# ccuchengwei/LongReadSelfCorrect

Measured on NVIDIA B200. Metric: corrected Mbp/s (seed + FM-extend + DP/MSA fallback, default options), higher is better.
Workload: dtype int64+f64

## Files before the change

longreadselfcorrect_b200/csrc/fm_table.cuh:

```cuda
#ifndef PBSC_FM_TABLE_CUH
#define PBSC_FM_TABLE_CUH

#include <cuda_runtime.h>
#include <stdint.h>

namespace pbsc {

struct __align__(32) FmBlock
{
    uint32_t cnt[4];
    uint32_t bases[4];
};

struct __align__(32) PrefixEntry
{
    uint64_t fwd_lo, rvc_lo;
    uint32_t fwd_size, rvc_size;
    uint32_t pad[2];
};

struct FmTable
{
    const FmBlock* blocks;
    const uint32_t* dollar_pos;
// ... 42 lines not shown
__host__ __device__ __forceinline__ uint32_t count_dollars(const FmTable& t, uint64_t from, uint64_t to)
{
    uint32_t lo = 0, hi = t.n_dollar;
    while (lo < hi) { uint32_t m = (lo + hi) >> 1; if ((uint64_t)PBSC_LDG(t.dollar_pos + m) < from) lo = m + 1; else hi = m; }
    uint32_t a = lo;
    hi = t.n_dollar;
    while (lo < hi) { uint32_t m = (lo + hi) >> 1; if ((uint64_t)PBSC_LDG(t.dollar_pos + m) < to) lo = m + 1; else hi = m; }
    return lo - a;
}

__host__ __device__ __forceinline__ uint64_t occ(const FmTable& t, int c, uint64_t p)
{
    PBSC_OCC_TICK(1);
    const uint64_t blk = p >> 6;
    const uint32_t off = (uint32_t)p & 63u;
    const uint4* bp = reinterpret_cast<const uint4*>(t.blocks + blk);
    const uint4 cn = PBSC_LDG(bp);
    const uint4 bs = PBSC_LDG(bp + 1);
    uint32_t base = c == 0 ? cn.x : c == 1 ? cn.y : c == 2 ? cn.z : cn.w;
    const bool has_dollar = (cn.x >> 31) != 0;
    if (c == 0) base &= 0x7fffffffu;
    const uint64_t w0 = (uint64_t)bs.x | ((uint64_t)bs.y << 32);
    const uint64_t w1 = (uint64_t)bs.z | ((uint64_t)bs.w << 32);
    const uint64_t pat = 0x5555555555555555ull * (uint64_t)c;
    uint64_t x0 = w0 ^ pat, x1 = w1 ^ pat;
    uint64_t m0 = ~(x0 | (x0 >> 1)) & 0x5555555555555555ull;
    uint64_t m1 = ~(x1 | (x1 >> 1)) & 0x5555555555555555ull;
    if (off < 32) { m0 &= (1ull << (2 * off)) - 1ull; m1 = 0; }
    else { m1 &= (1ull << (2 * (off - 32))) - 1ull; }
    uint64_t r = (uint64_t)base + PBSC_POPCLL(m0) + PBSC_POPCLL(m1);
    if (c == 0 && has_dollar && off) r -= PBSC_POPCLL(PBSC_LDG(t.dollar_mask + blk) & ((1ull << off) - 1ull));
    return r;
}

__host__ __device__ __forceinline__ void occ4(const FmTable& t, uint64_t p, uint64_t r[4])
{
    PBSC_OCC_TICK(1);
    const uint64_t blk = p >> 6;
    const uint32_t off = (uint32_t)p & 63u;
    const uint4* bp = reinterpret_cast<const uint4*>(t.blocks + blk);
    const uint4 cn = PBSC_LDG(bp);
    const uint4 bs = PBSC_LDG(bp + 1);
    const uint64_t w0 = (uint64_t)bs.x | ((uint64_t)bs.y << 32);
    const uint64_t w1 = (uint64_t)bs.z | ((uint64_t)bs.w << 32);
    const uint64_t M = 0x5555555555555555ull;
    uint64_t k0, k1;
    if (off < 32) { k0 = ((1ull << (2 * off)) - 1ull) & M; k1 = 0; }
    else { k0 = M; k1 = ((1ull << (2 * (off - 32))) - 1ull) & M; }
    const uint64_t l0 = w0 & M, h0 = (w0 >> 1) & M, l1 = w1 & M, h1 = (w1 >> 1) & M;
    const uint32_t nT = PBSC_POPCLL(h0 & l0 & k0) + PBSC_POPCLL(h1 & l1 & k1);
    const uint32_t nG = PBSC_POPCLL(h0 & ~l0 & k0) + PBSC_POPCLL(h1 & ~l1 & k1);
    const uint32_t nC = PBSC_POPCLL(~h0 & l0 & k0) + PBSC_POPCLL(~h1 & l1 & k1);
    uint32_t nA = off - nT - nG - nC;
    if ((cn.x >> 31) && off) nA -= PBSC_POPCLL(PBSC_LDG(t.dollar_mask + blk) & ((1ull << off) - 1ull));
    r[0] = (uint64_t)(cn.x & 0x7fffffffu) + nA;
    r[1] = (uint64_t)cn.y + nC;
    r[2] = (uint64_t)cn.z + nG;
    r[3] = (uint64_t)cn.w + nT;
}

__host__ __device__ __forceinline__ void occ_pair(const FmTable& t, int c, uint64_t lo, uint64_t hi, uint64_t& a, uint64_t& b)
{
    if ((lo >> 6) != (hi >> 6)) { a = occ(t, c, lo); b = occ(t, c, hi); return; }
    PBSC_OCC_TICK(1);
    const uint64_t blk = lo >> 6;
    const uint32_t off_a = (uint32_t)lo & 63u, off_b = (uint32_t)hi & 63u;
// ... 106 lines not shown
```

longreadselfcorrect_b200/csrc/pbsc_extend_thread.cu:

```cuda
#include <cub/cub.cuh>
#include <stdlib.h>
#include <string.h>
#include <algorithm>
#include <chrono>
#include "pbsc_batch.cuh"
#include "pbsc_task.cuh"
#include "pbsc_dp.cuh"

namespace pbsc {

constexpr int TW_BLOCK = 128;
struct ReadState
{
    int32_t t, next, started, done, rstatus, firstType;
    int32_t srcEnd, srcEndBest, srcRepeat;
    uint32_t nPieces;
    int64_t srcLen;
    uint64_t plen;
    int32_t pending_trg;
    int32_t srcFreq;
    int32_t srcStart;
    uint32_t nLog;
    int32_t dpStatus0;
    uint32_t dpLen0;
// ... 168 lines not shown
                                              : (y < (uint32_t)(k + interval) ? pth[y - k] : trgS[y - k - interval]);
            v.q[x] = 3 - c;
        }
    }
    tw::setup_task(idx, P, v, qlen, (uint32_t)k, interval, trgLen, tk.out_cap);
}

#ifdef PBSC_STAGE_CLOCKS
#define PBSC_N_STAGE 24
__device__ unsigned long long g_stage_clk[PBSC_N_STAGE];
#define STAGE_BEGIN() long long stg_t = clock64(); unsigned long long stg_acc[12] = {0, 0, 0, 0, 0, 0, 0, 0, 0, 0, 0, 0}
#define STAGE_MARK(i) do { const long long stg_n = clock64(); stg_acc[i] += (unsigned long long)(stg_n - stg_t); stg_t = stg_n; } while (0)
#define STAGE_COUNT(i, v) do { const unsigned stg_v = __reduce_add_sync(FULL, (unsigned)(v)); stg_acc[i] += stg_v; } while (0)
#define STAGE_END() do { if ((threadIdx.x & 31) == 0) for (int stg_i = 0; stg_i < 12; stg_i++) atomicAdd(&g_stage_clk[stg_i], stg_acc[stg_i]); } while (0)
#else
#define STAGE_BEGIN()
#define STAGE_MARK(i)
#define STAGE_COUNT(i, v)
#define STAGE_END()
#endif

__device__ __forceinline__ void
walk_levels_body(const FmIndexDev& idx, const ExtParamsDev& P, uint8_t* scratch, size_t stride,
                   unsigned long long* counter, uint64_t n_items, const uint32_t* __restrict__ list, WalkTask* tasks, uint8_t* recpool,
                   const uint64_t* __restrict__ rec_off, uint64_t pend_base, uint64_t pend_cap, uint8_t* outpool, uint64_t minSA,
                   unsigned long long* walk_counter, uint32_t* heavy_list, unsigned int* n_heavy, uint32_t* nodepool,
                   unsigned long long* pool_used, uint64_t pool_cap, tw::Caps caps, const unsigned int* n_items_dev, int last_pass, int owners)
{
    const bool owner = (int)(threadIdx.x & 31) < owners;
    const size_t tid = (((size_t)blockIdx.x * blockDim.x + threadIdx.x) >> 5) * (size_t)owners + (threadIdx.x & 31);
    __shared__ tw::Lane lanes_all[TW_BLOCK];
    tw::Lane* ctx = lanes_all + (threadIdx.x & ~31u);
    tw::Lane& S = ctx[threadIdx.x & 31];
    const tw::Layout Y = tw::make_layout(P.node_cap, caps);
    uint8_t* const my_scratch = scratch + (owner ? tid : 0) * stride;
    if (n_items_dev) n_items = *n_items_dev;
    S.status = 0; S.n = 0;
    WalkTask* tk = nullptr;
    tw::SetupHdr* hdr = nullptr;
    constexpr int REFILL_BATCH = 1;
    bool active = false, ended = false, exhausted = !owner;
    unsigned long long done = 0;
    STAGE_BEGIN();
    for (;;)
    {
        const unsigned waiting = __ballot_sync(FULL, !active && !exhausted);
        const unsigned walking = __ballot_sync(FULL, active);
        if (waiting && (__popc(waiting) >= REFILL_BATCH || !walking))
        {
            if (ended)
            {
                uint32_t mlen = 0;
                int st = tw::finish_walk(S, Y, P, hdr, nodepool, pool_used, pool_cap, last_pass != 0, outpool + tk->out_off, tk->out_cap, &mlen);
                if (st == PBSC_WALK_HEAVY && last_pass) st = PBSC_OVF_TREE;
                tk->out_len = st == 1 ? mlen : 0;
                tk->status = st;
                if (st == PBSC_WALK_HEAVY) heavy_list[atomicAdd(n_heavy, 1u)] = (uint32_t)(tk - tasks);
                ended = false;
            }
            if (!active && !exhausted)
            {
                for (;;)
                {
                    const unsigned long long it = atomicAdd(counter, 1ull);
                    if (it >= n_items) { exhausted = true; break; }
                    const uint64_t ti = list ? list[it] : it;
                    tk = &tasks[ti];
// ... 5 lines not shown
                    tw::begin_walk(S, Y, P, my_scratch, v, minSA);
                    hdr = v.hdr;
                    active = true;
                    done++;
                    break;
                }
            }
        }
        if (__all_sync(FULL, !active)) break;
        STAGE_MARK(0);
        const bool lv = active && tw::walk_continues(S, P);
        {
            const bool need = lv && tw::needs_refine(S);
            STAGE_COUNT(9, 1u);
            STAGE_COUNT(10, lv ? 1u : 0u);
            STAGE_COUNT(11, lv ? S.n : 0u);
            tw::refine_pool(idx, Y, ctx, need ? S.n : 0u);
            if (need) S.curK = S.maxOverlap;
        }
        STAGE_MARK(1);
        if (lv)
        {
            tw::filter_leaves(S, Y);
            S.thr = S.phase == 2 ? S.minSA - 1 : S.minSA;
        }
        STAGE_MARK(2);
        tw::pool_run(lv ? S.n : 0u, [&](int owner_lane, uint32_t i) { tw::probe_leaf(idx, Y, ctx[owner_lane], i); });
        STAGE_MARK(3);
        uint32_t m = 0, sel = 0;
        bool go = false;
        if (lv)
        {
            m = tw::adopt_children(S, Y);
            if (S.status == 0) go = tw::level_middle(S, Y, P, m, sel);
        }
        STAGE_MARK(4);
        if (__any_sync(FULL, sel != 0))
        {
            tw::pool_run(sel, [&](int owner_lane, uint32_t i) { tw::select_leaf(idx, Y, ctx[owner_lane], i); });
            if (sel) tw::level_select(S, P);
            tw::pool_run(sel, [&](int owner_lane, uint32_t i) { tw::reselect_leaf(idx, Y, ctx[owner_lane], i); });
        }
        STAGE_MARK(5);
        tw::pool_run(go ? m : 0u, [&](int owner_lane, uint32_t j) { tw::prune_leaf(P, Y, ctx[owner_lane], j); });
        STAGE_MARK(6);
        bool check_term = false;
        if (go) { S.level++; check_term = S.curLen >= S.minLength; }
        tw::pool_run(check_term ? m : 0u, [&](int owner_lane, uint32_t j) { tw::term_leaf(Y, ctx[owner_lane], j); });
        STAGE_MARK(7);
        if (go) tw::finish_level(S, Y, P, m, check_term);
        if (active && !tw::walk_continues(S, P)) { active = false; ended = true; }
        STAGE_MARK(8);
    }
    STAGE_END();
    if (done) atomicAdd(walk_counter, done);
}

template <int MINB>
__global__ void __launch_bounds__(TW_BLOCK, MINB)
walk_levels_kernel(const __grid_constant__ FmIndexDev idx, const __grid_constant__ ExtParamsDev P, uint8_t* scratch, size_t stride,
                   unsigned long long* counter, uint64_t n_items, const uint32_t* __restrict__ list, WalkTask* tasks, uint8_t* recpool,
                   const uint64_t* __restrict__ rec_off, uint64_t pend_base, uint64_t pend_cap, uint8_t* outpool, uint64_t minSA,
                   unsigned long long* walk_counter, uint32_t* heavy_list, unsigned int* n_heavy, uint32_t* nodepool,
                   unsigned long long* pool_used, uint64_t pool_cap, tw::Caps caps, const unsigned int* n_items_dev, int last_pass, int owners)
{
    walk_levels_body(idx, P, scratch, stride, counter, n_items, list, tasks, recpool, rec_off, pend_base, pend_cap, outpool, minSA, walk_counter,
                     heavy_list, n_heavy, nodepool, pool_used, pool_cap, caps, n_items_dev, last_pass, owners);
// ... 610 lines not shown
```

longreadselfcorrect_b200/csrc/pbsc_walk_thread.cuh:

```cuda
#ifndef PBSC_WALK_THREAD_CUH
#define PBSC_WALK_THREAD_CUH

#include "pbsc_walk.cuh"

namespace pbsc {
namespace tw {

struct Caps { uint32_t old_cap, new_cap, rings, res; };
#define PBSC_WALK_HEAVY (-102)

struct Layout
{
    uint32_t bank1, rings, nodes, res, ringStack, list0, list1;
    uint32_t node_cap;
    Caps cap;
};

__host__ __device__ inline uint32_t pow2_ceil(uint32_t x) { uint32_t p = 1; while (p < x) p <<= 1; return p; }

__host__ __device__ inline size_t thread_scratch_bytes(uint32_t node_cap, Caps c)
{
    size_t b = 0;
    b += sizeof(Leaf) * (size_t)(2 * c.new_cap);
    b += sizeof(double) * (size_t)c.rings * RING_LEN;
// ... 15 lines not shown
    y.ringStack = (uint32_t)p; p += align_up(c.rings, 16);
    y.list0 = (uint32_t)p; p += align_up(c.new_cap, 16);
    y.list1 = (uint32_t)p;
    y.node_cap = node_cap; y.cap = c;
    return y;
}

struct __align__(16) Lane
{
    uint8_t* base;
    const uint16_t* start4; const uint16_t* pos4; const uint8_t* q;
    const uint64_t* hash; const uint64_t* sF; const uint64_t* sR;
    const Interval* termF; const Interval* termR;
    double minErr;
    uint32_t curLen, curK, maxLength, minLength, maxIndel, minSA, thr;
    uint32_t qlen, k, maxOverlap, trgLen, nTerm, n9F, n9R, n5, nNodes, nRes, level, hashMask, nFree, nFresh, phase, n;
    uint32_t selLB, selExtra, selK;
    int selMx[3];
    int status;
    uint8_t dup, flip, selNew, pad;
};
static_assert(sizeof(Lane) == 208, "Lane: 208 bytes of shared memory per thread");

__device__ __forceinline__ Leaf* old_bank(const Lane& s, const Layout& y) { return (Leaf*)(s.base + (s.flip ? y.bank1 : 0u)); }
__device__ __forceinline__ Leaf* new_bank(const Lane& s, const Layout& y) { return (Leaf*)(s.base + (s.flip ? 0u : y.bank1)); }
__device__ __forceinline__ uint8_t* old_list(const Lane& s, const Layout& y) { return s.base + (s.flip ? y.list1 : y.list0); }
__device__ __forceinline__ uint8_t* new_list(const Lane& s, const Layout& y) { return s.base + (s.flip ? y.list0 : y.list1); }
__device__ __forceinline__ double* rings_of(const Lane& s, const Layout& y) { return (double*)(s.base + y.rings); }
__device__ __forceinline__ uint32_t* nodes_of(const Lane& s, const Layout& y) { return (uint32_t*)(s.base + y.nodes); }
__device__ __forceinline__ WalkResult* res_of(const Lane& s, const Layout& y) { return (WalkResult*)(s.base + y.res); }
__device__ __forceinline__ uint8_t* ring_stack(const Lane& s, const Layout& y) { return s.base + y.ringStack; }

static __device__ __noinline__ Interval update1(const FmTable& t, Interval iv, int c) { return update_interval(t, iv, c); }
static __device__ __noinline__ void occ4_ool(const FmTable& t, uint64_t p, uint64_t r[4]) { occ4(t, p, r); }
__device__ __forceinline__ void leaf_copy(Leaf* dst, const Leaf* src)
{
    const uint4* s4 = reinterpret_cast<const uint4*>(src);
    uint4* d4 = reinterpret_cast<uint4*>(dst);
    #pragma unroll
    for (int x = 0; x < (int)(sizeof(Leaf) / 16); x++) d4[x] = s4[x];
}

template <class Get>
__device__ __forceinline__ void both_strands(const FmIndexDev& idx, Get get, int K, Interval& f, Interval& r)
{
    int j;
    if (idx.prefix != nullptr && K >= idx.k0)
    {
        uint64_t key = 0;
        #pragma unroll 1
        for (int i = 0; i < idx.k0; i++) key |= (uint64_t)get(i) << (2 * i);
        prefix_lookup(idx, key, f, r);
        j = idx.k0;
    }
    else
    {
        const int c = get(0);
        f = init_interval(idx.t[PBSC_RBWT], c);
        r = init_interval(idx.t[PBSC_BWT], 3 - c);
        j = 1;
    }
    #pragma unroll 1
    for (; j < K && (f.valid() || r.valid()); j++)
    {
        const int c = get(j);
        if (f.valid()) f = update1(idx.t[PBSC_RBWT], f, c);
        if (r.valid()) r = update1(idx.t[PBSC_BWT], r, 3 - c);
    }
}

template <class F>
__device__ __forceinline__ void pool_run(uint32_t cnt, F f)
{
    __syncwarp();
// ... 27 lines not shown
}

__device__ __forceinline__ void ring_release(Lane& S, const Layout& Y, uint32_t slot) { ring_stack(S, Y)[S.nFree++] = (uint8_t)slot; }
__device__ __forceinline__ int ring_take(Lane& S, const Layout& Y)
{
    if (S.nFree) return (int)ring_stack(S, Y)[--S.nFree];
    return S.nFresh < Y.cap.rings ? (int)S.nFresh++ : -1;
}

__device__ __forceinline__ void refine_pool(const FmIndexDev& idx, const Layout& Y, const Lane* ctx, uint32_t cnt)
{
    pool_run(cnt, [&](int owner, uint32_t i) {
        const Lane& c = ctx[owner];
        Leaf* L = old_bank(c, Y) + old_list(c, Y)[i];
        const uint64_t rhi = L->rt_hi, rlo = L->rt_lo;
        const int K = (int)c.maxOverlap;
        Interval f, r;
        both_strands(idx, [&](int j) { return tail_base(rhi, rlo, K - 1 - j); }, K, f, r);
        L->f_lo = f.lo; L->f_hi = f.hi; L->r_lo = r.lo; L->r_hi = r.hi;
    });
}

__device__ __forceinline__ bool insufficient(const ExtParamsDev& P, const Leaf* bank, const uint8_t* list, uint32_t cnt)
{
    uint32_t high = 0;
    #pragma unroll 1
    for (uint32_t j = 0; j < cnt; j++) high += bank[list[j]].kmerFreq > P.high_freq_thr;
    if (high == 0) return true;
    if (high <= 2 && cnt >= 5) return true;
    if (high <= 1 && cnt >= 3) return true;
    return false;
}

static __device__ __noinline__ uint32_t eval4(const int freq[4], uint64_t totalcount, int maxfreq, uint32_t match5, uint32_t tailCount, uint64_t cutoffSA)
{
    uint32_t mask = 0;
    if (maxfreq <= 0) return 0;
    const bool isHomopolymer = tailCount >= 3;
    const bool isRepeat = maxfreq > 100, isHighlyRepeat = maxfreq > 150, isLowlyRepeat = maxfreq > 50;
    const bool isLowCoverage = totalcount >= cutoffSA + 2;
    #pragma unroll 1
    for (int b = 0; b < 4; b++)
    {
        const uint64_t kmerFreq = (uint64_t)(int64_t)freq[b];
        const bool isMatchedBy5mer = (match5 >> b) & 1;
        const bool isFreqPass = kmerFreq >= cutoffSA;
        int p, q;
        if (isMatchedBy5mer && isHighlyRepeat) { p = 1; q = 8; }
        else if (isMatchedBy5mer && isLowlyRepeat) { p = 1; q = 5; }
        else if (isFreqPass) { p = 1; q = 4; }
        else if (isLowCoverage) { p = 3; q = 5; }
        else { p = 2; q = 1; }
        if (isHomopolymer && isRepeat) { if (p * 10 < 3 * q) { p = 3; q = 10; } }
        else if (isHomopolymer) { if (p * 5 < 3 * q) { p = 3; q = 5; } }
        if ((int64_t)freq[b] * q >= (int64_t)p * maxfreq) mask |= 1u << b;
    }
    return mask;
}

__device__ __forceinline__ uint32_t match5_mask(const Lane& c, uint32_t tail4)
{
    const int64_t lo = max((int64_t)c.curLen - (int64_t)c.maxIndel, (int64_t)0);
    const int64_t hi = min((int64_t)c.curLen + (int64_t)c.maxIndel, (int64_t)c.n5 - 1);
    uint32_t mask = 0;
    const uint32_t e1 = c.start4[tail4 + 1];
    #pragma unroll 1
    for (uint32_t e = c.start4[tail4]; e < e1; e++)
    {
        const int64_t p = c.pos4[e];
        if (p >= lo && p <= hi) mask |= 1u << c.q[p + 4];
    }
    return mask;
}

static __device__ __noinline__ void filter_leaves(Lane& S, const Layout& Y)
{
    Leaf* oldL = old_bank(S, Y);
    uint8_t* list = old_list(S, Y);
    double minErr = 1.0;
    #pragma unroll 1
    for (uint32_t i = 0; i < S.n; i++) minErr = fmin(minErr, oldL[list[i]].local_err);
    uint32_t w = 0;
    #pragma unroll 1
    for (uint32_t i = 0; i < S.n; i++)
    {
        const Leaf& L = oldL[list[i]];
        const double diff = __dsub_rn(L.local_err, minErr);
        const bool drop = (diff > 0.05 && S.curLen > (uint32_t)(RING_LEN / 2)) || (diff > 0.1 && S.curLen > 15);
        if (drop) { ring_release(S, Y, L.ring); continue; }
        if (w != i) list[w] = list[i];
        w++;
    }
    S.n = w;
    S.minErr = minErr;
}

__device__ __forceinline__ void probe_leaf(const FmIndexDev& idx, const Layout& Y, const Lane& c, uint32_t i)
{
    Leaf* parent = old_bank(c, Y) + old_list(c, Y)[i];
    uint64_t fl[4], fh[4], rl[4], rh[4];
    const uint64_t pf_lo = parent->f_lo, pf_hi = parent->f_hi, pr_lo = parent->r_lo, pr_hi = parent->r_hi;
    const bool fV = pf_hi > pf_lo, rV = pr_hi > pr_lo;
    if (fV) { occ4_ool(idx.t[PBSC_RBWT], pf_lo, fl); occ4_ool(idx.t[PBSC_RBWT], pf_hi, fh); }
    if (rV) { occ4_ool(idx.t[PBSC_BWT], pr_lo, rl); occ4_ool(idx.t[PBSC_BWT], pr_hi, rh); }
    int freq[4];
    Interval pf[4], pr[4];
    uint64_t total = 0;
    int mx = 0;
    uint32_t match5 = 0;
    const uint64_t p_rt_hi = parent->rt_hi;
    const uint32_t near5 = match5_mask(c, (uint32_t)(p_rt_hi >> 56));
    #pragma unroll 1
    for (int b = 0; b < 4; b++)
    {
        if (fV) { pf[b].lo = idx.t[PBSC_RBWT].C[b] + fl[b]; pf[b].hi = idx.t[PBSC_RBWT].C[b] + fh[b]; }
        else { pf[b].lo = pf_lo; pf[b].hi = pf_hi; }
        if (rV) { pr[b].lo = idx.t[PBSC_BWT].C[3 - b] + rl[3 - b]; pr[b].hi = idx.t[PBSC_BWT].C[3 - b] + rh[3 - b]; }
        else { pr[b].lo = pr_lo; pr[b].hi = pr_hi; }
        freq[b] = (int)((int64_t)pf[b].size() + (int64_t)pr[b].size());
        total += (uint64_t)(int64_t)freq[b];
        mx = max(mx, freq[b]);
        if ((pf[b].valid() || pr[b].valid()) && ((near5 >> b) & 1)) match5 |= 1u << b;
    }
    const uint32_t p_tailCount = parent->tailCount;
    uint32_t mask = eval4(freq, total, mx, match5, p_tailCount, (uint64_t)c.thr);
    if (!mask && parent->local_err == c.minErr && c.n > 1) mask = eval4(freq, total, mx, match5, p_tailCount, (uint64_t)c.thr - 1);
    parent->aux = mask;
    if (!mask) return;
    const uint32_t p_tailLetter = parent->tailLetter;
    const uint64_t p_rt_lo = parent->rt_lo;
    Leaf* newL = new_bank(c, Y);
    #pragma unroll 1
    for (int b = 0; b < 4; b++)
    {
        if (!((mask >> b) & 1)) continue;
        Leaf* ch = newL + 4 * i + b;
        leaf_copy(ch, parent);
        ch->f_lo = pf[b].lo; ch->f_hi = pf[b].hi; ch->r_lo = pr[b].lo; ch->r_hi = pr[b].hi;
        ch->kmerFreq = freq[b];
        uint64_t th = p_rt_hi, tl = p_rt_lo;
        tail_push(th, tl, b);
        ch->rt_hi = th; ch->rt_lo = tl;
        if (p_tailLetter == (uint32_t)b) ch->tailCount = p_tailCount + 1; else { ch->tailLetter = (uint8_t)b; ch->tailCount = 1; }
        ch->alive = 1;
        ch->aux = 0;
    }
}

static __device__ __noinline__ uint32_t adopt_children(Lane& S, const Layout& Y)
{
    Leaf* oldL = old_bank(S, Y);
    Leaf* newL = new_bank(S, Y);
    const uint8_t* list = old_list(S, Y);
    uint8_t* cl = new_list(S, Y);
    uint32_t* nodes = nodes_of(S, Y);
    const uint32_t n = S.n;
    uint32_t total = 0;
    #pragma unroll 1
    for (uint32_t i = 0; i < n; i++) total += __popc(oldL[list[i]].aux);
    if (total == 0) return 0;
    if (S.nNodes + total > Y.node_cap) { S.status = PBSC_WALK_HEAVY; return 0; }
    uint32_t m = 0;
    #pragma unroll 1
    for (uint32_t i = 0; i < n; i++)
    {
        const Leaf& parent = oldL[list[i]];
        const uint32_t mask = parent.aux;
        const uint32_t p_ring = parent.ring;
        if (!mask) { ring_release(S, Y, p_ring); continue; }
        const uint32_t p_node = parent.node;
        uint32_t j = 0;
        #pragma unroll 1
        for (int b = 0; b < 4; b++)
        {
            if (!((mask >> b) & 1)) continue;
            Leaf* c = newL + 4 * i + b;
            const uint32_t node = S.nNodes++;
            c->node = node;
            nodes[node] = (p_node << 2) | (uint32_t)b;
            if (j > 0)
            {
                const int slot = ring_take(S, Y);
                if (slot < 0) { S.status = PBSC_WALK_HEAVY; return 0; }
                c->ring = (uint16_t)slot;
                c->aux = p_ring + 1;
            }
            cl[m++] = (uint8_t)(4 * i + b);
            j++;
        }
    }
    return m;
}

__device__ __forceinline__ int hash_find(const Lane& c, uint32_t key)
{
    uint32_t h = (key * 2654435761u) & c.hashMask;
    #pragma unroll 1
    for (;;)
    {
        const uint64_t e = c.hash[h];
        if (e == ~0ull) return -1;
        if ((uint32_t)(e >> 32) == key) return (int)(uint32_t)e;
        h = (h + 1) & c.hashMask;
    }
}

static __device__ __noinline__ double ddiv_ool(double a, double b) { return __ddiv_rn(a, b); }
static __device__ __noinline__ uint64_t urem_ool(uint64_t a, uint64_t b) { return a % b; }

__device__ __forceinline__ void prune_leaf(const ExtParamsDev& P, const Layout& Y, const Lane& c, uint32_t j)
{
    const uint64_t seedSize = (uint64_t)P.seed_size;
    const uint64_t curLen = c.curLen;
    const uint64_t currSeedIdx = curLen - seedSize;
    const uint64_t indelOffset = seedSize + c.maxIndel;
    const uint64_t smallSeedIdx = currSeedIdx <= indelOffset ? 0 : currSeedIdx - indelOffset;
    const uint64_t largeSeedIdx = (currSeedIdx + indelOffset) >= ((uint64_t)c.qlen - seedSize) ? ((uint64_t)c.qlen - seedSize) : currSeedIdx + indelOffset;
    const uint32_t keyMask = (1u << (2 * P.seed_size)) - 1u;
    Leaf& L = new_bank(c, Y)[new_list(c, Y)[j]];
    bool found = false;
    const uint64_t d = curLen - (uint64_t)L.lastOverlapLen;
    if (d > seedSize || d <= 1)
    {
        const uint64_t preSeedIdx = L.lastSeedIdx;
        const uint64_t seedIdxOffset = (uint64_t)L.lastOverlapLen < curLen - seedSize ? seedSize : curLen - (uint64_t)L.lastOverlapLen;
        const uint64_t startSeedIdx = max(smallSeedIdx, (uint64_t)L.lastSeedIdx + seedIdxOffset);
        const bool fV = L.f_hi > L.f_lo, rV = L.r_hi > L.r_lo;
        const uint32_t keyF = (uint32_t)(L.rt_hi >> (64 - 2 * P.seed_size));
        if (!c.dup)
        {
            if (fV || rV)
            {
                const int p = hash_find(c, keyF);
                if (p >= 0 && (uint64_t)p >= startSeedIdx && (uint64_t)p <= largeSeedIdx)
                {
                    if (abs(p - (int)currSeedIdx) < 10000) L.lastSeedIdx = (uint32_t)p;
                    L.lastOverlapLen = (uint32_t)curLen;
                    found = true;
                }
            }
        }
        else
        {
            uint32_t nf = 0, nr = 0, gf = 0, gr = 0;
            if (fV) gf = group_find(c.sF, c.n9F, keyF, nf);
            if (rV) gr = group_find(c.sR, c.n9R, keyMask - keyF, nr);
            int minIdxDiff = 10000;
            const uint32_t lim = max(nf, nr);
            #pragma unroll 1
            for (uint32_t i = 0; i < lim; i++)
            {
                uint64_t v = 0;
                bool hit = false;
                if (i < nf) { v = (uint32_t)c.sF[gf + i]; hit = v >= startSeedIdx && v <= largeSeedIdx; }
                if (!hit && i < nr) { v = (uint32_t)c.sR[gr + i]; hit = v >= startSeedIdx && v <= largeSeedIdx; }
                if (hit)
                {
                    const int diff = abs((int)v - (int)currSeedIdx);
                    if (diff < minIdxDiff) { L.lastSeedIdx = (uint32_t)v; minIdxDiff = diff; }
                    L.lastOverlapLen = (uint32_t)curLen;
                    found = true;
                }
            }
        }
        if (found)
        {
            L.totalSeeds++;
            if (currSeedIdx + (uint64_t)(int64_t)L.seedOff - preSeedIdx > seedSize) L.redeem = __dadd_rn(L.redeem, P.redeem_a);
            L.seedOff = (int)L.lastSeedIdx - (int)currSeedIdx;
        }
        else
        {
            const uint64_t v = currSeedIdx + (uint64_t)(int64_t)L.seedOff - (uint64_t)L.lastSeedIdx;
            if (urem_ool(v, seedSize) == 1) {  }
            else if (v > seedSize - 1) L.redeem = __dadd_rn(L.redeem, P.redeem_b);
        }
    }
    else L.redeem = __dadd_rn(L.redeem, P.redeem_b);
    double matchedLen = __dsub_rn(__dadd_rn((double)L.totalSeeds, (double)seedSize), 1.0);
    matchedLen = __dadd_rn(matchedLen, L.redeem);
    const double totalLen = (double)curLen;
    double err = ddiv_ool(__dsub_rn(totalLen, matchedLen), totalLen);
    double* ring = rings_of(c, Y) + (size_t)L.ring * RING_LEN;
    if (L.aux)
    {
        const double* src = rings_of(c, Y) + (size_t)(L.aux - 1) * RING_LEN;
        const int have = min((int)c.level, RING_LEN);
        #pragma unroll 4
        for (int x = 0; x < have; x++) ring[x] = src[x];
        L.aux = 0;
    }
    ring[c.level % RING_LEN] = err;
    L.global_err = err;
    if (c.level + 1 >= (uint32_t)RING_LEN)
    {
        const double old = ring[(c.level + 1) % RING_LEN];
        err = ddiv_ool(__dsub_rn(__dmul_rn(err, totalLen), __dmul_rn(old, __dsub_rn(totalLen, (double)RING_LEN))), (double)RING_LEN);
    }
    L.local_err = err;
    if (err > P.walk_error_rate) L.alive = 0;
}

__device__ __forceinline__ void term_leaf(const Layout& Y, const Lane& c, uint32_t j)
{
    Leaf& L = new_bank(c, Y)[new_list(c, Y)[j]];
    if (!L.alive) { L.aux = 0; return; }
    const bool fV = L.f_hi > L.f_lo, rV = L.r_hi > L.r_lo;
    const uint64_t f_lo = L.f_lo, f_hi = L.f_hi, r_lo = L.r_lo, r_hi = L.r_hi;
    int ilast = -1;
    #pragma unroll 1
    for (int i = max(L.res_second, 0); i < (int)c.nTerm; i++)
    {
        const Interval tf = c.termF[i], tr = c.termR[i];
        const bool ft = fV && tf.valid() && f_lo >= tf.lo && f_hi <= tf.hi;
        const bool rt = rV && tr.valid() && r_lo >= tr.lo && r_hi <= tr.hi;
        if (ft || rt) ilast = i;
    }
    L.aux = (uint32_t)(ilast + 1);
}

static __device__ __noinline__ void finish_level(Lane& S, const Layout& Y, const ExtParamsDev& P, uint32_t m, bool check_term)
{
    Leaf* newL = new_bank(S, Y);
    uint8_t* cl = new_list(S, Y);
    WalkResult* res = res_of(S, Y);
    if (check_term)
    {
        #pragma unroll 1
        for (uint32_t j = 0; j < m; j++)
        {
            Leaf& L = newL[cl[j]];
            if (!L.alive || L.aux == 0) continue;
            const int ilast = (int)L.aux - 1;
            int slot = L.res_first;
            if (slot == -1)
            {
                if (S.nRes >= Y.cap.res) { S.status = PBSC_WALK_HEAVY; return; }
                slot = (int)++S.nRes;
            }
            WalkResult r; r.err = L.global_err; r.node = L.node; r.i = ilast; r.depth = (uint32_t)S.curLen; r.pad = 0;
            res[slot - 1] = r;
            L.res_first = slot; L.res_second = ilast;
        }
    }
// ... 236 lines not shown
        const int ch = tail_base(hi, lo, 0);
        a = init_interval(idx.t[PBSC_BWT], ch);
        b = init_interval(idx.t[PBSC_RBWT], 3 - ch);
        d = 1;
    }
    #pragma unroll 1
    for (; d < LB && (a.valid() || b.valid()); d++)
    {
        const int ch = tail_base(hi, lo, d);
        if (a.valid()) a = update1(idx.t[PBSC_BWT], a, ch);
        if (b.valid()) b = update1(idx.t[PBSC_RBWT], b, 3 - ch);
    }
    atomicMax(&c.selMx[0], (int)((int64_t)a.size() + (int64_t)b.size()));
    #pragma unroll 1
    for (int e = 1; e <= extra; e++)
    {
        const int ch = tail_base(hi, lo, LB - 1 + e);
        if (a.valid()) a = update1(idx.t[PBSC_BWT], a, ch);
        if (b.valid()) b = update1(idx.t[PBSC_RBWT], b, 3 - ch);
        atomicMax(&c.selMx[e], (int)((int64_t)a.size() + (int64_t)b.size()));
    }
}

__device__ __forceinline__ void reselect_leaf(const FmIndexDev& idx, const Layout& Y, const Lane& c, uint32_t i)
{
    Leaf& L = (c.selNew ? new_bank(c, Y) : old_bank(c, Y))[(c.selNew ? new_list(c, Y) : old_list(c, Y))[i]];
    const uint64_t hi = L.rt_hi, lo = L.rt_lo;
    const int K = (int)c.selK;
    Interval f, r;
    both_strands(idx, [&](int j) { return tail_base(hi, lo, K - 1 - j); }, K, f, r);
    L.f_lo = f.lo; L.f_hi = f.hi; L.r_lo = r.lo; L.r_hi = r.hi;
}

static __device__ __noinline__ bool level_middle(Lane& S, const Layout& Y, const ExtParamsDev& P, uint32_t m, uint32_t& sel)
{
    uint32_t cnt = 0;
    sel = 0;
    if (m > 0)
    {
        S.curLen++;
        S.curK++;
        S.phase = 0;
        if (insufficient(P, new_bank(S, Y), new_list(S, Y), m)) { S.selNew = 1; cnt = m; }
    }
    else if (S.phase == 0) { S.selNew = 0; cnt = S.n; S.phase = 1; }
    else if (S.phase == 1) { S.phase = 2; return false; }
    else { S.n = 0; return false; }
    if (cnt)
    {
        const uint32_t LB = max(S.curK - 2, (uint32_t)P.min_overlap);
        S.selLB = LB; S.selExtra = S.curK - LB;
        S.selMx[0] = S.selMx[1] = S.selMx[2] = 0;
        sel = cnt;
    }
    return m > 0;
}

__device__ __forceinline__ void level_select(Lane& S, const ExtParamsDev& P)
{
    const uint32_t LB = S.selLB, UB = LB + S.selExtra;
    uint32_t R = UB;
    if (S.selMx[0] - P.freq_int[LB] < 5) R = LB;
    else
    {
        #pragma unroll 1
        for (uint32_t e = 1; e <= S.selExtra; e++) if (S.selMx[e] - P.freq_int[LB + e] < 5) { R = LB + e; break; }
    }
    S.selK = R;
    S.curK = R;
}

#define PBSC_TASK_MATERIALIZE 2

static __device__ __noinline__ int finish_walk(Lane& S, const Layout& Y, const ExtParamsDev& P, SetupHdr* hdr, uint32_t* nodepool, unsigned long long* pool_used,
                                               uint64_t pool_cap, bool direct, uint8_t* out, uint32_t outCap, uint32_t* outLen)
{
    if (S.status) return S.status;
    const WalkResult* res = res_of(S, Y);
    const uint32_t* nodes = nodes_of(S, Y);
    if (S.nRes > 0)
    {
        double best = 1.0;
        int bi = -1;
        #pragma unroll 1
        for (uint32_t i = 0; i < S.nRes; i++) { const double e = res[i].err; if (e < best) { best = e; bi = (int)i; } }
        if (bi < 0) return PBSC_WALK_NO_PATH;
        const WalkResult r = res[bi];
        if (direct)
// ... 61 lines not shown
```

Before: 82.28.

## Vectorize Leaf accesses as uint4 words and hoist FM sector loads

Rewrites leaf probing, child creation, seed checking and termination checks to read and write the Leaf struct as 16-byte uint4 words instead of scalar fields, and builds child leaves directly from parent words instead of copying then patching. FM block sectors for both interval endpoints are now loaded before the popcount work so the two loads can be in flight together. The change also moves the layout computation into shared memory, computed once per block, and packs level_middle's outputs into one return value. These edits aim to cut local/global memory transactions and register spills, but they rely on a hardcoded field layout, guarded by static_asserts, and the ring copy now moves pairs of doubles, which may copy one extra element.

```diff
diff --git a/longreadselfcorrect_b200/csrc/fm_table.cuh b/longreadselfcorrect_b200/csrc/fm_table.cuh
--- a/longreadselfcorrect_b200/csrc/fm_table.cuh
+++ b/longreadselfcorrect_b200/csrc/fm_table.cuh
@@ -98,6 +98,45 @@
     if (c == 0 && has_dollar && off) r -= PBSC_POPCLL(PBSC_LDG(t.dollar_mask + blk) & ((1ull << off) - 1ull));
     return r;
 }
+
+struct FmSector { uint4 cn, bs; };
+
+__host__ __device__ __forceinline__ FmSector load_sector(const FmTable& t, uint64_t p)
+{
+    PBSC_OCC_TICK(1);
+    const uint4* bp = reinterpret_cast<const uint4*>(t.blocks + (p >> 6));
+    FmSector s;
+    s.cn = PBSC_LDG(bp);
+    s.bs = PBSC_LDG(bp + 1);
+    return s;
+}
+
+__host__ __device__ __forceinline__ uint4 occ4_sector(const FmTable& t, uint64_t p, const FmSector& s)
+{
+    const uint64_t blk = p >> 6;
+    const uint32_t off = (uint32_t)p & 63u;
+    const uint4 cn = s.cn, bs = s.bs;
+    const uint64_t w0 = (uint64_t)bs.x | ((uint64_t)bs.y << 32);
+    const uint64_t w1 = (uint64_t)bs.z | ((uint64_t)bs.w << 32);
+    const uint64_t M = 0x5555555555555555ull;
+    uint64_t k0, k1;
+    if (off < 32) { k0 = ((1ull << (2 * off)) - 1ull) & M; k1 = 0; }
+    else { k0 = M; k1 = ((1ull << (2 * (off - 32))) - 1ull) & M; }
+    const uint64_t l0 = w0 & M, h0 = (w0 >> 1) & M, l1 = w1 & M, h1 = (w1 >> 1) & M;
+    const uint32_t nT = PBSC_POPCLL(h0 & l0 & k0) + PBSC_POPCLL(h1 & l1 & k1);
+    const uint32_t nG = PBSC_POPCLL(h0 & ~l0 & k0) + PBSC_POPCLL(h1 & ~l1 & k1);
+    const uint32_t nC = PBSC_POPCLL(~h0 & l0 & k0) + PBSC_POPCLL(~h1 & l1 & k1);
+    uint32_t nA = off - nT - nG - nC;
+    if ((cn.x >> 31) && off) nA -= PBSC_POPCLL(PBSC_LDG(t.dollar_mask + blk) & ((1ull << off) - 1ull));
+    uint4 r;
+    r.x = (cn.x & 0x7fffffffu) + nA;
+    r.y = cn.y + nC;
+    r.z = cn.z + nG;
+    r.w = cn.w + nT;
+    return r;
+}
+
+__host__ __device__ __forceinline__ uint4 occ4v(const FmTable& t, uint64_t p) { return occ4_sector(t, p, load_sector(t, p)); }
 
 __host__ __device__ __forceinline__ void occ4(const FmTable& t, uint64_t p, uint64_t r[4])
 {
diff --git a/longreadselfcorrect_b200/csrc/pbsc_extend_thread.cu b/longreadselfcorrect_b200/csrc/pbsc_extend_thread.cu
--- a/longreadselfcorrect_b200/csrc/pbsc_extend_thread.cu
+++ b/longreadselfcorrect_b200/csrc/pbsc_extend_thread.cu
@@ -224,7 +224,10 @@
     __shared__ tw::Lane lanes_all[TW_BLOCK];
     tw::Lane* ctx = lanes_all + (threadIdx.x & ~31u);
     tw::Lane& S = ctx[threadIdx.x & 31];
-    const tw::Layout Y = tw::make_layout(P.node_cap, caps);
+    __shared__ tw::Layout lay;
+    if (threadIdx.x == 0) lay = tw::make_layout(P.node_cap, caps);
+    __syncthreads();
+    const tw::Layout& Y = lay;
     uint8_t* const my_scratch = scratch + (owner ? tid : 0) * stride;
     if (n_items_dev) n_items = *n_items_dev;
     S.status = 0; S.n = 0;
@@ -296,7 +299,7 @@
         if (lv)
         {
             m = tw::adopt_children(S, Y);
-            if (S.status == 0) go = tw::level_middle(S, Y, P, m, sel);
+            if (S.status == 0) { const uint32_t r = tw::level_middle(S, Y, P, m); go = r & 1u; sel = r >> 1; }
         }
         STAGE_MARK(4);
         if (__any_sync(FULL, sel != 0))
diff --git a/longreadselfcorrect_b200/csrc/pbsc_walk_thread.cuh b/longreadselfcorrect_b200/csrc/pbsc_walk_thread.cuh
--- a/longreadselfcorrect_b200/csrc/pbsc_walk_thread.cuh
+++ b/longreadselfcorrect_b200/csrc/pbsc_walk_thread.cuh
@@ -71,14 +71,19 @@
 __device__ __forceinline__ uint8_t* ring_stack(const Lane& s, const Layout& y) { return s.base + y.ringStack; }
 
 static __device__ __noinline__ Interval update1(const FmTable& t, Interval iv, int c) { return update_interval(t, iv, c); }
-static __device__ __noinline__ void occ4_ool(const FmTable& t, uint64_t p, uint64_t r[4]) { occ4(t, p, r); }
-__device__ __forceinline__ void leaf_copy(Leaf* dst, const Leaf* src)
-{
-    const uint4* s4 = reinterpret_cast<const uint4*>(src);
-    uint4* d4 = reinterpret_cast<uint4*>(dst);
-    #pragma unroll
-    for (int x = 0; x < (int)(sizeof(Leaf) / 16); x++) d4[x] = s4[x];
-}
+static __device__ __noinline__ uint4 occ4_ool(const FmTable& t, uint64_t p, FmSector s) { return occ4_sector(t, p, s); }
+
+__device__ __forceinline__ uint32_t comp(uint4 v, int b) { return b == 0 ? v.x : b == 1 ? v.y : b == 2 ? v.z : v.w; }
+__device__ __forceinline__ uint64_t lo64(uint4 v) { return (uint64_t)v.x | ((uint64_t)v.y << 32); }
+__device__ __forceinline__ uint64_t hi64(uint4 v) { return (uint64_t)v.z | ((uint64_t)v.w << 32); }
+__device__ __forceinline__ uint4 u4(uint64_t a, uint64_t b) { return make_uint4((uint32_t)a, (uint32_t)(a >> 32), (uint32_t)b, (uint32_t)(b >> 32)); }
+
+__device__ __forceinline__ const uint4* words(const Leaf* L) { return reinterpret_cast<const uint4*>(L); }
+__device__ __forceinline__ uint4* words(Leaf* L) { return reinterpret_cast<uint4*>(L); }
+__device__ __forceinline__ uint32_t ring_tl_alive(uint32_t ring, uint32_t tailLetter, uint32_t alive) { return (ring & 0xffffu) | (tailLetter << 16) | (alive << 24); }
+static_assert(offsetof(Leaf, redeem) == 32 && offsetof(Leaf, global_err) == 48 && offsetof(Leaf, rt_lo) == 64 && offsetof(Leaf, totalSeeds) == 80 &&
+              offsetof(Leaf, res_second) == 96 && offsetof(Leaf, ring) == 108 && offsetof(Leaf, tailLetter) == 110 && offsetof(Leaf, alive) == 111 &&
+              offsetof(Leaf, aux) == 112, "the word layout above follows Leaf");
 
 template <class Get>
 __device__ __forceinline__ void both_strands(const FmIndexDev& idx, Get get, int K, Interval& f, Interval& r)
@@ -172,7 +177,7 @@
     return false;
 }
 
-static __device__ __noinline__ uint32_t eval4(const int freq[4], uint64_t totalcount, int maxfreq, uint32_t match5, uint32_t tailCount, uint64_t cutoffSA)
+static __device__ __noinline__ uint32_t eval4(int4 freq4, uint64_t totalcount, int maxfreq, uint32_t match5, uint32_t tailCount, uint64_t cutoffSA)
 {
     uint32_t mask = 0;
     if (maxfreq <= 0) return 0;
@@ -182,7 +187,8 @@
     #pragma unroll 1
     for (int b = 0; b < 4; b++)
     {
-        const uint64_t kmerFreq = (uint64_t)(int64_t)freq[b];
+        const int fb = b == 0 ? freq4.x : b == 1 ? freq4.y : b == 2 ? freq4.z : freq4.w;
+        const uint64_t kmerFreq = (uint64_t)(int64_t)fb;
         const bool isMatchedBy5mer = (match5 >> b) & 1;
         const bool isFreqPass = kmerFreq >= cutoffSA;
         int p, q;
@@ -193,7 +199,7 @@
         else { p = 2; q = 1; }
         if (isHomopolymer && isRepeat) { if (p * 10 < 3 * q) { p = 3; q = 10; } }
         else if (isHomopolymer) { if (p * 5 < 3 * q) { p = 3; q = 5; } }
-        if ((int64_t)freq[b] * q >= (int64_t)p * maxfreq) mask |= 1u << b;
+        if ((int64_t)fb * q >= (int64_t)p * maxfreq) mask |= 1u << b;
     }
     return mask;
 }
@@ -238,52 +244,65 @@
 __device__ __forceinline__ void probe_leaf(const FmIndexDev& idx, const Layout& Y, const Lane& c, uint32_t i)
 {
     Leaf* parent = old_bank(c, Y) + old_list(c, Y)[i];
-    uint64_t fl[4], fh[4], rl[4], rh[4];
-    const uint64_t pf_lo = parent->f_lo, pf_hi = parent->f_hi, pr_lo = parent->r_lo, pr_hi = parent->r_hi;
+    const uint4* pw = words(parent);
+    const uint4 w0 = pw[0], w1 = pw[1];
+    const uint64_t pf_lo = lo64(w0), pf_hi = hi64(w0), pr_lo = lo64(w1), pr_hi = hi64(w1);
     const bool fV = pf_hi > pf_lo, rV = pr_hi > pr_lo;
-    if (fV) { occ4_ool(idx.t[PBSC_RBWT], pf_lo, fl); occ4_ool(idx.t[PBSC_RBWT], pf_hi, fh); }
-    if (rV) { occ4_ool(idx.t[PBSC_BWT], pr_lo, rl); occ4_ool(idx.t[PBSC_BWT], pr_hi, rh); }
+    const FmTable& TF = idx.t[PBSC_RBWT];
+    const FmTable& TR = idx.t[PBSC_BWT];
+    uint4 fl = make_uint4(0, 0, 0, 0), fh = fl, rl = fl, rh = fl;
+    if (fV) { const FmSector a = load_sector(TF, pf_lo), b = load_sector(TF, pf_hi); fl = occ4_ool(TF, pf_lo, a); fh = occ4_ool(TF, pf_hi, b); }
+    if (rV) { const FmSector a = load_sector(TR, pr_lo), b = load_sector(TR, pr_hi); rl = occ4_ool(TR, pr_lo, a); rh = occ4_ool(TR, pr_hi, b); }
+    const uint4 w3 = pw[3], w5 = pw[5];
+    const uint64_t p_rt_hi = hi64(w3);
+    const uint32_t near5 = match5_mask(c, (uint32_t)(p_rt_hi >> 56));
+    auto child_iv = [&](int b, uint64_t& flo, uint64_t& fhi, uint64_t& rlo, uint64_t& rhi) {
+        if (fV) { flo = TF.C[b] + comp(fl, b); fhi = TF.C[b] + comp(fh, b); } else { flo = pf_lo; fhi = pf_hi; }
+        if (rV) { rlo = TR.C[3 - b] + comp(rl, 3 - b); rhi = TR.C[3 - b] + comp(rh, 3 - b); } else { rlo = pr_lo; rhi = pr_hi; }
+    };
     int freq[4];
-    Interval pf[4], pr[4];
     uint64_t total = 0;
     int mx = 0;
     uint32_t match5 = 0;
-    const uint64_t p_rt_hi = parent->rt_hi;
-    const uint32_t near5 = match5_mask(c, (uint32_t)(p_rt_hi >> 56));
-    #pragma unroll 1
+    #pragma unroll
     for (int b = 0; b < 4; b++)
     {
-        if (fV) { pf[b].lo = idx.t[PBSC_RBWT].C[b] + fl[b]; pf[b].hi = idx.t[PBSC_RBWT].C[b] + fh[b]; }
-        else { pf[b].lo = pf_lo; pf[b].hi = pf_hi; }
-        if (rV) { pr[b].lo = idx.t[PBSC_BWT].C[3 - b] + rl[3 - b]; pr[b].hi = idx.t[PBSC_BWT].C[3 - b] + rh[3 - b]; }
-        else { pr[b].lo = pr_lo; pr[b].hi = pr_hi; }
-        freq[b] = (int)((int64_t)pf[b].size() + (int64_t)pr[b].size());
+        uint64_t flo, fhi, rlo, rhi;
+        child_iv(b, flo, fhi, rlo, rhi);
+        freq[b] = (int)((int64_t)(fhi - flo) + (int64_t)(rhi - rlo));
         total += (uint64_t)(int64_t)freq[b];
         mx = max(mx, freq[b]);
-        if ((pf[b].valid() || pr[b].valid()) && ((near5 >> b) & 1)) match5 |= 1u << b;
-    }
-    const uint32_t p_tailCount = parent->tailCount;
-    uint32_t mask = eval4(freq, total, mx, match5, p_tailCount, (uint64_t)c.thr);
-    if (!mask && parent->local_err == c.minErr && c.n > 1) mask = eval4(freq, total, mx, match5, p_tailCount, (uint64_t)c.thr - 1);
+        if ((fhi > flo || rhi > rlo) && ((near5 >> b) & 1)) match5 |= 1u << b;
+    }
+    const int4 freq4 = make_int4(freq[0], freq[1], freq[2], freq[3]);
+    const uint32_t p_tailCount = w5.y;
+    uint32_t mask = eval4(freq4, total, mx, match5, p_tailCount, (uint64_t)c.thr);
+    if (!mask && parent->local_err == c.minErr && c.n > 1) mask = eval4(freq4, total, mx, match5, p_tailCount, (uint64_t)c.thr - 1);
     parent->aux = mask;
     if (!mask) return;
-    const uint32_t p_tailLetter = parent->tailLetter;
-    const uint64_t p_rt_lo = parent->rt_lo;
-    Leaf* newL = new_bank(c, Y);
+    const uint4 w2 = pw[2], w4 = pw[4], w6 = pw[6];
+    const uint32_t p_tailLetter = (w6.w >> 16) & 0xffu;
+    const uint64_t p_rt_lo = lo64(w4);
+    uint4* const kids = words(new_bank(c, Y) + 4 * i);
     #pragma unroll 1
     for (int b = 0; b < 4; b++)
     {
         if (!((mask >> b) & 1)) continue;
-        Leaf* ch = newL + 4 * i + b;
-        leaf_copy(ch, parent);
-        ch->f_lo = pf[b].lo; ch->f_hi = pf[b].hi; ch->r_lo = pr[b].lo; ch->r_hi = pr[b].hi;
-        ch->kmerFreq = freq[b];
+        uint64_t flo, fhi, rlo, rhi;
+        child_iv(b, flo, fhi, rlo, rhi);
+        const int fq = b == 0 ? freq4.x : b == 1 ? freq4.y : b == 2 ? freq4.z : freq4.w;
         uint64_t th = p_rt_hi, tl = p_rt_lo;
         tail_push(th, tl, b);
-        ch->rt_hi = th; ch->rt_lo = tl;
-        if (p_tailLetter == (uint32_t)b) ch->tailCount = p_tailCount + 1; else { ch->tailLetter = (uint8_t)b; ch->tailCount = 1; }
-        ch->alive = 1;
-        ch->aux = 0;
+        const uint32_t tc = p_tailLetter == (uint32_t)b ? p_tailCount + 1 : 1;
+        uint4* d = kids + 8 * b;
+        d[0] = u4(flo, fhi);
+        d[1] = u4(rlo, rhi);
+        d[2] = w2;
+        d[3] = make_uint4(w3.x, w3.y, (uint32_t)th, (uint32_t)(th >> 32));
+        d[4] = make_uint4((uint32_t)tl, (uint32_t)(tl >> 32), w4.z, w4.w);
+        d[5] = make_uint4(w5.x, tc, w5.z, w5.w);
+        d[6] = make_uint4(w6.x, (uint32_t)fq, w6.z, ring_tl_alive(w6.w, (uint32_t)b, 1u));
+        d[7] = make_uint4(0, 0, 0, 0);
     }
 }
 
@@ -306,9 +325,10 @@
     {
         const Leaf& parent = oldL[list[i]];
         const uint32_t mask = parent.aux;
-        const uint32_t p_ring = parent.ring;
+        const uint2 nr = *reinterpret_cast<const uint2*>(&parent.node);
+        const uint32_t p_ring = nr.y & 0xffffu;
         if (!mask) { ring_release(S, Y, p_ring); continue; }
-        const uint32_t p_node = parent.node;
+        const uint32_t p_node = nr.x;
         uint32_t j = 0;
         #pragma unroll 1
         for (int b = 0; b < 4; b++)
@@ -316,15 +336,16 @@
             if (!((mask >> b) & 1)) continue;
             Leaf* c = newL + 4 * i + b;
             const uint32_t node = S.nNodes++;
-            c->node = node;
             nodes[node] = (p_node << 2) | (uint32_t)b;
+            uint32_t ring = p_ring;
             if (j > 0)
             {
                 const int slot = ring_take(S, Y);
                 if (slot < 0) { S.status = PBSC_WALK_HEAVY; return 0; }
-                c->ring = (uint16_t)slot;
+                ring = (uint32_t)slot;
                 c->aux = p_ring + 1;
             }
+            *reinterpret_cast<uint2*>(&c->node) = make_uint2(node, ring_tl_alive(ring, (uint32_t)b, 1u));
             cl[m++] = (uint8_t)(4 * i + b);
             j++;
         }
@@ -358,14 +379,20 @@
     const uint64_t largeSeedIdx = (currSeedIdx + indelOffset) >= ((uint64_t)c.qlen - seedSize) ? ((uint64_t)c.qlen - seedSize) : currSeedIdx + indelOffset;
     const uint32_t keyMask = (1u << (2 * P.seed_size)) - 1u;
     Leaf& L = new_bank(c, Y)[new_list(c, Y)[j]];
+    uint4* const lw = words(&L);
+    const uint4 w2 = lw[2], w4 = lw[4], w5 = lw[5];
+    uint32_t lastSeedIdx = w4.z, lastOverlapLen = w4.w, totalSeeds = w5.x;
+    int32_t seedOff = (int32_t)w5.z;
+    double redeem = __longlong_as_double((long long)lo64(w2));
     bool found = false;
-    const uint64_t d = curLen - (uint64_t)L.lastOverlapLen;
+    const uint64_t d = curLen - (uint64_t)lastOverlapLen;
     if (d > seedSize || d <= 1)
     {
-        const uint64_t preSeedIdx = L.lastSeedIdx;
-        const uint64_t seedIdxOffset = (uint64_t)L.lastOverlapLen < curLen - seedSize ? seedSize : curLen - (uint64_t)L.lastOverlapLen;
-        const uint64_t startSeedIdx = max(smallSeedIdx, (uint64_t)L.lastSeedIdx + seedIdxOffset);
-        const bool fV = L.f_hi > L.f_lo, rV = L.r_hi > L.r_lo;
+        const uint64_t preSeedIdx = lastSeedIdx;
+        const uint64_t seedIdxOffset = (uint64_t)lastOverlapLen < curLen - seedSize ? seedSize : curLen - (uint64_t)lastOverlapLen;
+        const uint64_t startSeedIdx = max(smallSeedIdx, (uint64_t)lastSeedIdx + seedIdxOffset);
+        const uint4 w0 = lw[0], w1 = lw[1];
+        const bool fV = hi64(w0) > lo64(w0), rV = hi64(w1) > lo64(w1);
         const uint32_t keyF = (uint32_t)(L.rt_hi >> (64 - 2 * P.seed_size));
         if (!c.dup)
         {
@@ -374,8 +401,8 @@
                 const int p = hash_find(c, keyF);
                 if (p >= 0 && (uint64_t)p >= startSeedIdx && (uint64_t)p <= largeSeedIdx)
                 {
-                    if (abs(p - (int)currSeedIdx) < 10000) L.lastSeedIdx = (uint32_t)p;
-                    L.lastOverlapLen = (uint32_t)curLen;
+                    if (abs(p - (int)currSeedIdx) < 10000) lastSeedIdx = (uint32_t)p;
+                    lastOverlapLen = (uint32_t)curLen;
                     found = true;
                 }
             }
@@ -397,37 +424,42 @@
                 if (hit)
                 {
                     const int diff = abs((int)v - (int)currSeedIdx);
-                    if (diff < minIdxDiff) { L.lastSeedIdx = (uint32_t)v; minIdxDiff = diff; }
-                    L.lastOverlapLen = (uint32_t)curLen;
+                    if (diff < minIdxDiff) { lastSeedIdx = (uint32_t)v; minIdxDiff = diff; }
+                    lastOverlapLen = (uint32_t)curLen;
                     found = true;
                 }
             }
         }
         if (found)
         {
-            L.totalSeeds++;
-            if (currSeedIdx + (uint64_t)(int64_t)L.seedOff - preSeedIdx > seedSize) L.redeem = __dadd_rn(L.redeem, P.redeem_a);
-            L.seedOff = (int)L.lastSeedIdx - (int)currSeedIdx;
+            totalSeeds++;
+            if (currSeedIdx + (uint64_t)(int64_t)seedOff - preSeedIdx > seedSize) redeem = __dadd_rn(redeem, P.redeem_a);
+            seedOff = (int)lastSeedIdx - (int)currSeedIdx;
+            *reinterpret_cast<uint2*>(&L.lastSeedIdx) = make_uint2(lastSeedIdx, lastOverlapLen);
+            lw[5] = make_uint4(totalSeeds, w5.y, (uint32_t)seedOff, w5.w);
         }
         else
         {
-            const uint64_t v = currSeedIdx + (uint64_t)(int64_t)L.seedOff - (uint64_t)L.lastSeedIdx;
+            const uint64_t v = currSeedIdx + (uint64_t)(int64_t)seedOff - (uint64_t)lastSeedIdx;
             if (urem_ool(v, seedSize) == 1) {  }
-            else if (v > seedSize - 1) L.redeem = __dadd_rn(L.redeem, P.redeem_b);
+            else if (v > seedSize - 1) redeem = __dadd_rn(redeem, P.redeem_b);
         }
     }
-    else L.redeem = __dadd_rn(L.redeem, P.redeem_b);
-    double matchedLen = __dsub_rn(__dadd_rn((double)L.totalSeeds, (double)seedSize), 1.0);
-    matchedLen = __dadd_rn(matchedLen, L.redeem);
+    else redeem = __dadd_rn(redeem, P.redeem_b);
+    double matchedLen = __dsub_rn(__dadd_rn((double)totalSeeds, (double)seedSize), 1.0);
+    matchedLen = __dadd_rn(matchedLen, redeem);
     const double totalLen = (double)curLen;
     double err = ddiv_ool(__dsub_rn(totalLen, matchedLen), totalLen);
-    double* ring = rings_of(c, Y) + (size_t)L.ring * RING_LEN;
-    if (L.aux)
-    {
-        const double* src = rings_of(c, Y) + (size_t)(L.aux - 1) * RING_LEN;
+    const uint32_t ringAlive = reinterpret_cast<const uint32_t*>(lw)[27];
+    const uint32_t aux = reinterpret_cast<const uint32_t*>(lw)[28];
+    double* ring = rings_of(c, Y) + (size_t)(ringAlive & 0xffffu) * RING_LEN;
+    if (aux)
+    {
+        const double2* src = reinterpret_cast<const double2*>(rings_of(c, Y) + (size_t)(aux - 1) * RING_LEN);
+        double2* dst = reinterpret_cast<double2*>(ring);
         const int have = min((int)c.level, RING_LEN);
         #pragma unroll 4
-        for (int x = 0; x < have; x++) ring[x] = src[x];
+        for (int x = 0; x < (have + 1) / 2; x++) dst[x] = src[x];
         L.aux = 0;
     }
     ring[c.level % RING_LEN] = err;
@@ -437,19 +469,22 @@
         const double old = ring[(c.level + 1) % RING_LEN];
         err = ddiv_ool(__dsub_rn(__dmul_rn(err, totalLen), __dmul_rn(old, __dsub_rn(totalLen, (double)RING_LEN))), (double)RING_LEN);
     }
-    L.local_err = err;
+    lw[2] = u4((uint64_t)__double_as_longlong(redeem), (uint64_t)__double_as_longlong(err));
     if (err > P.walk_error_rate) L.alive = 0;
 }
 
 __device__ __forceinline__ void term_leaf(const Layout& Y, const Lane& c, uint32_t j)
 {
     Leaf& L = new_bank(c, Y)[new_list(c, Y)[j]];
-    if (!L.alive) { L.aux = 0; return; }
-    const bool fV = L.f_hi > L.f_lo, rV = L.r_hi > L.r_lo;
-    const uint64_t f_lo = L.f_lo, f_hi = L.f_hi, r_lo = L.r_lo, r_hi = L.r_hi;
+    const uint4* lw = words(&L);
+    const uint4 w6 = lw[6];
+    if (!(w6.w >> 24)) { L.aux = 0; return; }
+    const uint4 w0 = lw[0], w1 = lw[1];
+    const uint64_t f_lo = lo64(w0), f_hi = hi64(w0), r_lo = lo64(w1), r_hi = hi64(w1);
+    const bool fV = f_hi > f_lo, rV = r_hi > r_lo;
     int ilast = -1;
     #pragma unroll 1
-    for (int i = max(L.res_second, 0); i < (int)c.nTerm; i++)
+    for (int i = max((int32_t)w6.x, 0); i < (int)c.nTerm; i++)
     {
         const Interval tf = c.termF[i], tr = c.termR[i];
         const bool ft = fV && tf.valid() && f_lo >= tf.lo && f_hi <= tf.hi;
@@ -752,10 +787,9 @@
     L.f_lo = f.lo; L.f_hi = f.hi; L.r_lo = r.lo; L.r_hi = r.hi;
 }
 
-static __device__ __noinline__ bool level_middle(Lane& S, const Layout& Y, const ExtParamsDev& P, uint32_t m, uint32_t& sel)
+static __device__ __noinline__ uint32_t level_middle(Lane& S, const Layout& Y, const ExtParamsDev& P, uint32_t m)
 {
     uint32_t cnt = 0;
-    sel = 0;
     if (m > 0)
     {
         S.curLen++;
@@ -764,16 +798,15 @@
         if (insufficient(P, new_bank(S, Y), new_list(S, Y), m)) { S.selNew = 1; cnt = m; }
     }
     else if (S.phase == 0) { S.selNew = 0; cnt = S.n; S.phase = 1; }
-    else if (S.phase == 1) { S.phase = 2; return false; }
-    else { S.n = 0; return false; }
+    else if (S.phase == 1) { S.phase = 2; return 0; }
+    else { S.n = 0; return 0; }
     if (cnt)
     {
         const uint32_t LB = max(S.curK - 2, (uint32_t)P.min_overlap);
         S.selLB = LB; S.selExtra = S.curK - LB;
         S.selMx[0] = S.selMx[1] = S.selMx[2] = 0;
-        sel = cnt;
-    }
-    return m > 0;
+    }
+    return (cnt << 1) | (m > 0 ? 1u : 0u);
 }
 
 __device__ __forceinline__ void level_select(Lane& S, const ExtParamsDev& P)
```

Result: faster. 87.63 (median of 6 runs) (+6.5%).
